# fulliu/lc

Measured on AMD Instinct MI355X. Metric: poses/sec (cov-loss fwd+bwd + weighted PnP), B=256 N=64, 1/2/4/8 MI355X, higher is better.
Workload: dtype f64; 1 GPU; configs[1]: synthetic B=256 N=64 2D-3D correspondences per GPU, HIP weighted-PnP + cov-loss; global_batch=256, n_points=64, launch=graph_region, launch_agreed_by_all_ranks=True

## Files before the change

### lc_amd/csrc/lc_common.h

```cpp
#pragma once
#include <hip/hip_runtime.h>

namespace lc {

#ifndef LC_NT_GRAD_STORES
#define LC_NT_GRAD_STORES 1
#endif
typedef float lc_v4f_t __attribute__((ext_vector_type(4)));
__device__ __forceinline__ void store_stream4(float* q, float a, float b, float c, float d) {
#if LC_NT_GRAD_STORES
    lc_v4f_t r = {a, b, c, d};
    __builtin_nontemporal_store(r, reinterpret_cast<lc_v4f_t*>(q));
#else
    *reinterpret_cast<float4*>(q) = make_float4(a, b, c, d);
#endif
}


constexpr int kWave = 64;

constexpr int kDppQuadXor1 = 0xB1;
constexpr int kDppQuadXor2 = 0x4E;
constexpr int kDppIdentity = 0xE4;
constexpr int kDppRowMirror = 0x140;
// ... 210 lines not shown
#pragma unroll
    for (int k = 0; k < K; ++k) v[k] = tot[k];
}

constexpr int kSplitMaxParts = 8;
#ifndef LC_SPLIT_WAIT_US
#define LC_SPLIT_WAIT_US 2000
#endif
constexpr unsigned long long kSplitWaitTicks = 100ull * LC_SPLIT_WAIT_US;
__device__ __forceinline__ bool split_wait_expired(int polls, unsigned long long& t0) {
    if ((polls & 15) != 15) return false;
    const unsigned long long now = __builtin_amdgcn_s_memrealtime();
    if (t0 == 0) { t0 = now; return false; }
    return now - t0 > kSplitWaitTicks;
}
constexpr int kSplitRowWords = 64;
constexpr size_t kSplitPoseBytes = 2 * kSplitMaxParts * kSplitRowWords * sizeof(unsigned long long) + 128;
constexpr int kSplitLdsDoubles = 128 + 64 + 2;
constexpr int kSplitSerialLdsDoubles = 128 + 32 * kSplitMaxParts + 32;
struct SplitSum {
    unsigned long long* exch;
    unsigned* epoch;
    int G, part;
    unsigned base;
    unsigned seq;
    bool timed_out;
};
__device__ __forceinline__ unsigned* split_tail(void* region, size_t region_bytes) {
    return reinterpret_cast<unsigned*>(static_cast<char*>(region) + region_bytes - 128);
}
__device__ __forceinline__ SplitSum split_sum_enter(void* pose_region, int G, int part) {
    unsigned* epoch = split_tail(pose_region, kSplitPoseBytes);
    return SplitSum{reinterpret_cast<unsigned long long*>(pose_region), epoch, G, part, xcd_load(epoch), 0u, false};
}
__device__ __forceinline__ void split_sum_leave(const SplitSum& sx) {
    if (sx.timed_out) xcd_store(sx.epoch + 1, 1u);
    else if (sx.part == 0 && sx.seq > 0) xcd_store(sx.epoch, sx.base + sx.seq);
}
__device__ __forceinline__ bool split_rescue_enter(void* region, size_t region_bytes, bool redo, int tid, int threads) {
    unsigned* tail = split_tail(region, region_bytes);
    const bool dirty = xcd_load(tail + 1) != 0u;
    if (!dirty && !redo) return false;
    __syncthreads();
    if (dirty) {
        unsigned long long* w = static_cast<unsigned long long*>(region);
        for (size_t i = tid; i < (region_bytes - 128) / 8; i += threads) xcd_store(w + i, 0ull);
        if (tid < 2) xcd_store(tail + tid, 0u);
    }
    if (redo && tid == 0) xcd_store(tail + 2, xcd_load(tail + 2) + 1u);
    return redo;
}

template <int K>
__device__ __forceinline__ void block_sum_split(double (&v)[K], double* lds, int tid, int& phase, SplitSum& sx) {
    static_assert(K <= 32, "one reduce-scatter of 32");
    const int lane = tid & 63, wave = tid >> 6;
    double w[32];
#pragma unroll
    for (int k = 0; k < 32; ++k) w[k] = k < K ? v[k] : 0.0;
    wave_reduce_scatter16<32>(w, lane);
    double* part = lds;
    double* tot = lds + 128 + 32 * phase;
    int* arrived_ok = reinterpret_cast<int*>(lds + 192);
    phase ^= 1;
    if (sx.timed_out) {
#pragma unroll
        for (int k = 0; k < K; ++k) v[k] = 0.0;
        return;
    }
    if ((lane & 3) == 0) *reinterpret_cast<double2*>(part + 32 * wave + scatter16_base(lane, 2)) = make_double2(w[0], w[1]);
    __syncthreads();
    if (tid < 32) {
        const unsigned long long ticket = (unsigned long long)(sx.base + sx.seq + 1u) << 32;
        unsigned long long* rows = sx.exch + (size_t)(sx.seq & 1u) * (kSplitMaxParts * kSplitRowWords) + 2 * tid;
        {
            const unsigned long long bits = __builtin_bit_cast(unsigned long long, ((part[tid] + part[32 + tid]) + part[64 + tid]) + part[96 + tid]);
            unsigned long long* mine = rows + sx.part * kSplitRowWords;
            xcd_store(mine, ticket | (bits & 0xFFFFFFFFull));
            xcd_store(mine + 1, ticket | (bits >> 32));
        }
        unsigned long long lo[kSplitMaxParts], hi[kSplitMaxParts];
        bool ok = true;
        unsigned long long t0 = 0;
        for (int polls = 0;; ++polls) {
#pragma unroll
            for (int g = 0; g < kSplitMaxParts; ++g)
                if (g < sx.G) {
                    lo[g] = xcd_load(rows + g * kSplitRowWords);
                    hi[g] = xcd_load(rows + g * kSplitRowWords + 1);
                }
            unsigned long long late = 0;
#pragma unroll
            for (int g = 0; g < kSplitMaxParts; ++g)
                if (g < sx.G) late |= ((lo[g] ^ ticket) | (hi[g] ^ ticket)) >> 32;
            if (late == 0) break;
            if (split_wait_expired(polls, t0)) { ok = false; break; }
            __builtin_amdgcn_s_sleep(1);
        }
        double s = 0.0;
#pragma unroll
        for (int g = 0; g < kSplitMaxParts; ++g)
            if (g < sx.G) s += __builtin_bit_cast(double, (hi[g] << 32) | (lo[g] & 0xFFFFFFFFull));
        tot[tid] = s;
        if (!ok) *arrived_ok = 0;
    }
    __syncthreads();
    if (!*arrived_ok) sx.timed_out = true;
#pragma unroll
    for (int k = 0; k < K; ++k) v[k] = tot[k];
    ++sx.seq;
}

template <int K>
__device__ __forceinline__ void block_sum_parts_serial(double (&v)[K], double* lds, int tid, int g, int G) {
    static_assert(K <= 32, "one reduce-scatter of 32");
    const int lane = tid & 63, wave = tid >> 6;
    double w[32];
#pragma unroll
    for (int k = 0; k < 32; ++k) w[k] = k < K ? v[k] : 0.0;
    wave_reduce_scatter16<32>(w, lane);
    double* part = lds;
    double* rows = lds + 128;
    double* tot = lds + 128 + 32 * kSplitMaxParts;
    if ((lane & 3) == 0) *reinterpret_cast<double2*>(part + 32 * wave + scatter16_base(lane, 2)) = make_double2(w[0], w[1]);
    __syncthreads();
    if (tid < 32) {
        rows[32 * g + tid] = ((part[tid] + part[32 + tid]) + part[64 + tid]) + part[96 + tid];
        if (g == G - 1) {
            double s = 0.0;
            for (int h = 0; h < G; ++h) s += rows[32 * h + tid];
            tot[tid] = s;
        }
    }
    __syncthreads();
    if (g == G - 1) {
#pragma unroll
        for (int k = 0; k < K; ++k) v[k] = tot[k];
    }
}

#ifndef LC_HORNER_ASM
#define LC_HORNER_ASM 1
#endif
__device__ __forceinline__ double horner_step(double p, double z, double c) {
#if LC_HORNER_ASM
    double r;
    asm("v_fma_f64 %0, %1, %2, %3" : "=v"(r) : "v"(p), "v"(z), "v"(c));
    return r;
#else
    return __builtin_fma(p, z, c);
#endif
}

__device__ __forceinline__ void sincos_small(double x, double& s, double& c) {
    if (!(x < 1.0e4)) {
        sincos(x, &s, &c);
        return;
    }
    const double kf = __builtin_rint(x * 0.63661977236758134308);
    const int q = (int)kf;
    double r = __builtin_fma(-kf, 1.57079632673412561417e+00, x);
    r = __builtin_fma(-kf, 6.07710050650619224932e-11, r);
    r = __builtin_fma(-kf, 2.02226624879595063154e-21, r);
    const double z = r * r;
    double ps = horner_step(1.58969099521155010221e-10, z, -2.50507602534068634195e-08);
    ps = horner_step(ps, z, 2.75573137070700676789e-06);
    ps = horner_step(ps, z, -1.98412698298579493134e-04);
    ps = horner_step(ps, z, 8.33333333332248946124e-03);
    ps = horner_step(ps, z, -1.66666666666666324348e-01);
    const double sr = __builtin_fma(ps * z, r, r);
    double pc = horner_step(-1.13596475577881948265e-11, z, 2.08757232129817482790e-09);
    pc = horner_step(pc, z, -2.75573143513906633035e-07);
    pc = horner_step(pc, z, 2.48015872894767294178e-05);
    pc = horner_step(pc, z, -1.38888888888741095749e-03);
    pc = horner_step(pc, z, 4.16666666666666019037e-02);
    const double cr = __builtin_fma(pc * z, z, __builtin_fma(-0.5, z, 1.0));
    const double ss = (q & 1) ? cr : sr, cc = (q & 1) ? sr : cr;
    s = (q & 2) ? -ss : ss;
    c = ((q + 1) & 2) ? -cc : cc;
}

__device__ __forceinline__ double atan_ratio_pos(double s, double c) {
    const bool swap = s > c;
    const double a = swap ? c : s, b = swap ? s : c;
    double t = a * fast_rcp(b);
#pragma unroll
    for (int k = 0; k < 2; ++k) {
        const double h = fast_sqrt(__builtin_fma(t, t, 1.0));
        t = t * fast_rcp(1.0 + h);
    }
    const double w = t * t;
    double p = horner_step(-1.0 / 21.0, w, 1.0 / 19.0);
    p = horner_step(p, w, -1.0 / 17.0);
    p = horner_step(p, w, 1.0 / 15.0);
    p = horner_step(p, w, -1.0 / 13.0);
    p = horner_step(p, w, 1.0 / 11.0);
    p = horner_step(p, w, -1.0 / 9.0);
    p = horner_step(p, w, 1.0 / 7.0);
    p = horner_step(p, w, -1.0 / 5.0);
    p = horner_step(p, w, 1.0 / 3.0);
    const double at = 4.0 * __builtin_fma(-(p * w), t, t);
    return swap ? 1.57079632679489661923 - at : at;
}

__device__ __forceinline__ bool uniform(bool c) { return __builtin_amdgcn_ballot_w64(c) != 0ull; }

__host__ __device__ constexpr int tri6(int i, int j) { return i * 6 - (i * (i - 1)) / 2 + (j - i); }

}
```

### lc_amd/csrc/lc_fused_kernel.h

```cpp
#pragma once
#include "lc_loss_body.h"
#include "lc_pnp_body.h"

#ifndef LC_UNIT_PRIO
#define LC_UNIT_PRIO 1
#endif

#ifndef LC_UNIT_ATTR
#define LC_UNIT_ATTR
#endif

namespace lc {
namespace {

union __attribute__((aligned(16))) FusedShared {
    loss::LossShared loss;
    double bc[pnp::kPnpLdsDoubles<1>];
};

template <int WPS>
__global__ __launch_bounds__(64, WPS) LC_UNIT_ATTR void lc_pose_unit_kernel(const LossParams lp, const PnpParams pp) {
    __shared__ FusedShared sh;
    if ((int)blockIdx.x < pp.B) {
#if LC_UNIT_PRIO
        __builtin_amdgcn_s_setprio(3);
#endif
        pnp::solve_pose<true, 1>(pp, blockIdx.x, threadIdx.x, sh.bc);
    } else {
#ifndef LC_UNIT_NOLOSS
        loss::sample<true>(lp, (int)blockIdx.x - pp.B, sh.loss);
#endif
    }
}

}

int launch_pose_unit_latency(const LossParams& lp, const PnpParams& pp, int blocks, hipStream_t stream);

}
```

### lc_amd/csrc/lc_pnp.hip

```cpp
#include "lc_pnp_kernels.h"

namespace lc {
namespace {


#ifndef LC_BIG_LOWREG
#define LC_BIG_LOWREG 0
#endif
#if LC_BIG_LOWREG
template <bool OPTS = false>
__global__ __launch_bounds__(64, 3) void lc_pnp_lm_big_kernel(const PnpParams p) {
    __shared__ __attribute__((aligned(16))) double bc[pnp::kPnpLowregLdsDoubles];
    pnp::solve_pose_lowreg<OPTS>(p, blockIdx.x, threadIdx.x, bc);
}
#endif

template <bool REG, bool OPTS = false, int PPT = 0, bool TAIL = false>
__global__ __launch_bounds__(256) void lc_pnp_lm_wide_kernel(const PnpParams p) {
    __shared__ __attribute__((aligned(16))) double bc[pnp::kPnpLdsDoubles<4>];
    pnp::solve_pose<REG, 4, false, OPTS, PPT, TAIL>(p, blockIdx.x, threadIdx.x, bc);
}

__global__ __launch_bounds__(256) void lc_pnp_lm_chain_kernel(const PnpParams a, const PnpParams b, const int second_starts_from_first) {
    __shared__ __attribute__((aligned(16))) double bc[pnp::kPnpLdsDoubles<4>];
    __shared__ float refined[8];
    pnp::solve_pose<false, 4, false, true, 4>(a, (int)(blockIdx.x % (unsigned)a.B), threadIdx.x, bc, blockIdx.x < (unsigned)a.B, refined);
    __syncthreads();
    pnp::solve_pose<false, 4, false, true, 4>(b, blockIdx.x, threadIdx.x, bc, true, nullptr, second_starts_from_first ? refined : nullptr);
}

template <bool OPTS>
__global__ __launch_bounds__(256) void lc_pnp_lm_split_kernel(const PnpParams p) {
    __shared__ __attribute__((aligned(16))) double bc[kSplitLdsDoubles];
    const int xcd = (int)(blockIdx.x % 8u), j = (int)(blockIdx.x / 8u);
    const int part = j % p.split_parts, b = (j / p.split_parts) * 8 + xcd;
    if (b >= p.B) return;
    SplitSum sx = split_sum_enter(static_cast<char*>(p.split_ws) + (size_t)b * kSplitPoseBytes, p.split_parts, part);
    if (threadIdx.x == 0) *reinterpret_cast<int*>(bc + 192) = 1;
    pnp::solve_pose<false, 4, false, OPTS, 8, true, 1>(p, b, threadIdx.x, bc, part == 0, nullptr, nullptr, &sx);
    if (threadIdx.x == 0) split_sum_leave(sx);
}

template <bool OPTS>
__global__ __launch_bounds__(256) void lc_pnp_lm_split_rescue_kernel(const PnpParams p) {
    __shared__ __attribute__((aligned(16))) double bc[kSplitSerialLdsDoubles];
    const int b = (int)blockIdx.x;
    char* region = static_cast<char*>(p.split_ws) + (size_t)b * kSplitPoseBytes;
    const bool redo = __hip_atomic_load(p.rets + b, __ATOMIC_RELAXED, __HIP_MEMORY_SCOPE_AGENT) == kPnpPartNeverArrived;
    if (!split_rescue_enter(region, kSplitPoseBytes, redo, (int)threadIdx.x, 256)) return;
    SplitSum sx{nullptr, nullptr, p.split_parts, 0, 0u, 0u, false};
    pnp::solve_pose<false, 4, false, OPTS, 0, false, 2>(p, b, threadIdx.x, bc, true, nullptr, nullptr, &sx);
}

__global__ __launch_bounds__(64, 1) void lc_pnp_lm_trace_kernel(const PnpParams p) {
    __shared__ __attribute__((aligned(16))) double bc[pnp::kPnpLdsDoubles<1>];
    pnp::solve_pose<true, 1, true>(p, blockIdx.x, threadIdx.x, bc);
}
__global__ __launch_bounds__(256) void lc_pnp_lm_wide_trace_kernel(const PnpParams p) {
    __shared__ __attribute__((aligned(16))) double bc[pnp::kPnpLdsDoubles<4>];
    pnp::solve_pose<false, 4, true>(p, blockIdx.x, threadIdx.x, bc);
}

}

int launch_pnp_lm_trace(const PnpParams& p, hipStream_t stream) {
    if (p.B <= 0) return 0;
    if (p.Nmax <= 64) hipLaunchKernelGGL(lc_pnp_lm_trace_kernel, dim3(p.B), dim3(64), 0, stream, p);
    else hipLaunchKernelGGL(lc_pnp_lm_wide_trace_kernel, dim3(p.B), dim3(256), 0, stream, p);
    return hipGetLastError() == hipSuccess ? 0 : 2;
}

int launch_pnp_lm_chain(const PnpParams& a, const PnpParams& b, hipStream_t stream) {
    const auto wide4 = [](const PnpParams& p) { return p.Nmax > 256 && p.Nmax <= 1024; };
    const float* b_start = b.start ? b.start : b.states;
    const bool rows_match = b_start != a.states || b.pose_mod == a.B || (b.pose_mod == 0 && b.B == a.B);
    const bool first_is_safe = a.start != nullptr || b.B == a.B;
    if (a.B > 0 && b.B > 0 && a.Nmax <= 64 && b.Nmax <= 64 && b.B <= kLatencyGridMax && b.B % a.B == 0 && rows_match && first_is_safe)
        return launch_pnp_lm_chain_latency(a, b, b_start == a.states ? 1 : 0, stream);
    if (a.B > 0 && b.B > 0 && wide4(a) && wide4(b) && b.B % a.B == 0 && rows_match && first_is_safe) {
        hipLaunchKernelGGL(lc_pnp_lm_chain_kernel, dim3(b.B), dim3(256), 0, stream, a, b, b_start == a.states ? 1 : 0);
        return hipGetLastError() == hipSuccess ? 0 : 2;
    }
    if (int rc = launch_pnp_lm(a, stream)) return rc;
    return launch_pnp_lm(b, stream);
}

int device_compute_units() {
    static int cached[64] = {};
    int dev = 0, n = 0;
    if (hipGetDevice(&dev) != hipSuccess) return 0;
    if (dev >= 0 && dev < 64 && cached[dev]) return cached[dev];
    if (hipDeviceGetAttribute(&n, hipDeviceAttributeMultiprocessorCount, dev) != hipSuccess) return 0;
    if (dev >= 0 && dev < 64) cached[dev] = n;
    return n;
}
int split_parts_for(int units) {
    const int cus = device_compute_units();
    for (int parts = 8; parts >= 2; parts >>= 1)
        if ((long long)units * parts <= cus) return parts;
    return 1;
}

int pnp_split_parts(int B, int Nmax) {
    if (Nmax <= kSplitMinPoints || B <= 0) return 1;
    return split_parts_for((B + 7) / 8 * 8);
}
size_t pnp_split_workspace_bytes(int B, int Nmax) { return pnp_split_parts(B, Nmax) > 1 ? (size_t)B * kSplitPoseBytes : 0; }

int launch_pnp_lm(const PnpParams& p, hipStream_t stream) {
    if (p.B <= 0) return 0;
    if (p.split_ws && p.split_parts > 1) {
        const dim3 grid((unsigned)((p.B + 7) / 8 * 8 * p.split_parts));
        if (p.options || p.weight_mask || p.pose_mod > 0) {
            hipLaunchKernelGGL(lc_pnp_lm_split_kernel<true>, grid, dim3(256), 0, stream, p);
            hipLaunchKernelGGL(lc_pnp_lm_split_rescue_kernel<true>, dim3((unsigned)p.B), dim3(256), 0, stream, p);
        } else {
            hipLaunchKernelGGL(lc_pnp_lm_split_kernel<false>, grid, dim3(256), 0, stream, p);
            hipLaunchKernelGGL(lc_pnp_lm_split_rescue_kernel<false>, dim3((unsigned)p.B), dim3(256), 0, stream, p);
        }
        return hipGetLastError() == hipSuccess ? 0 : 2;
    }
    const bool big = p.B > kLatencyGridMax;
    if (p.options || p.weight_mask || p.pose_mod > 0) {
        if (p.Nmax <= 64) {
#if LC_BIG_LOWREG
            if (big) hipLaunchKernelGGL(lc_pnp_lm_big_kernel<true>, dim3(p.B), dim3(64), 0, stream, p);
#else
            if (big) hipLaunchKernelGGL((lc_pnp_lm_kernel<true, LC_BIG_WPS, true>), dim3(p.B), dim3(64), 0, stream, p);
#endif
            else return launch_pnp_lm_latency(p, stream);
        } else if (p.Nmax <= 256) {
            hipLaunchKernelGGL((lc_pnp_lm_wide_kernel<true, true>), dim3(p.B), dim3(256), 0, stream, p);
        } else if (p.Nmax <= 1024) {
            hipLaunchKernelGGL((lc_pnp_lm_wide_kernel<false, true, 4>), dim3(p.B), dim3(256), 0, stream, p);
        } else if (p.Nmax <= 2048) {
            hipLaunchKernelGGL((lc_pnp_lm_wide_kernel<false, true, 8>), dim3(p.B), dim3(256), 0, stream, p);
        } else {
            hipLaunchKernelGGL((lc_pnp_lm_wide_kernel<false, true, 16, true>), dim3(p.B), dim3(256), 0, stream, p);
        }
        return hipGetLastError() == hipSuccess ? 0 : 2;
    }
    if (p.Nmax <= 64) {
#if LC_BIG_LOWREG
        if (big) hipLaunchKernelGGL(lc_pnp_lm_big_kernel<false>, dim3(p.B), dim3(64), 0, stream, p);
#else
        if (big) hipLaunchKernelGGL((lc_pnp_lm_kernel<true, LC_BIG_WPS>), dim3(p.B), dim3(64), 0, stream, p);
#endif
        else return launch_pnp_lm_latency(p, stream);
    } else if (p.Nmax <= 256) {
        hipLaunchKernelGGL(lc_pnp_lm_wide_kernel<true>, dim3(p.B), dim3(256), 0, stream, p);
    } else if (p.Nmax <= 1024) {
        hipLaunchKernelGGL((lc_pnp_lm_wide_kernel<false, false, 4>), dim3(p.B), dim3(256), 0, stream, p);
    } else if (p.Nmax <= 2048) {
        hipLaunchKernelGGL((lc_pnp_lm_wide_kernel<false, false, 8>), dim3(p.B), dim3(256), 0, stream, p);
    } else {
        hipLaunchKernelGGL((lc_pnp_lm_wide_kernel<false, false, 16, true>), dim3(p.B), dim3(256), 0, stream, p);
    }
    return hipGetLastError() == hipSuccess ? 0 : 2;
}

}
```

### lc_amd/csrc/lc_pnp_body.h

```cpp
#pragma once
#include <cfloat>

#include "lc_common.h"
#include "lc_kernels.h"

#ifdef LC_STAMPS
#define LC_PSTAMP_DECL unsigned long long pst_[8] = {0, 0, 0, 0, 0, 0, 0, 0}, pt0_ = 0, pt1_ = 0
#define LC_PSTAMP_BEGIN()                                                                 \
    do {                                                                                  \
        __builtin_amdgcn_sched_barrier(0);                                                \
        asm volatile("s_memtime %0\n\ts_waitcnt lgkmcnt(0)" : "=s"(pt0_)::"memory");      \
        __builtin_amdgcn_sched_barrier(0);                                                \
    } while (0)
#define LC_PSTAMP(i)                                                                      \
    do {                                                                                  \
        __builtin_amdgcn_sched_barrier(0);                                                \
        asm volatile("s_memtime %0\n\ts_waitcnt lgkmcnt(0)" : "=s"(pt1_)::"memory");      \
        __builtin_amdgcn_sched_barrier(0);                                                \
        pst_[i] += pt1_ - pt0_;                                                           \
        pt0_ = pt1_;                                                                      \
    } while (0)
#else
#define LC_PSTAMP_DECL
#define LC_PSTAMP_BEGIN() do {} while (0)
#define LC_PSTAMP(i) do {} while (0)
#endif

#ifndef LC_WIDE_REG_SUM_REGS
#define LC_WIDE_REG_SUM_REGS 1
#endif
#ifndef LC_PNP_STREAM_SUM
#define LC_PNP_STREAM_SUM 1
#endif

namespace lc {
namespace pnp {

template <int NW>
constexpr int kPnpLdsDoubles = sum_bcast_lds_doubles<NW>(28);

struct Point {
    double X[3];
    double u, v;
    double a, b, c;
};

struct Rot {
    double R[9];
    double Jr[9];
};

__device__ __forceinline__ void make_rot(const double aa[3], Rot& o) {
    const double x = aa[0], y = aa[1], z = aa[2];
    const double th2 = x * x + y * y + z * z;
    const bool small = !(th2 > DBL_EPSILON);
    double th, ith;
    fast_sqrt_rsqrt(th2, th, ith);
    double s, c;
    sincos_small(th, s, c);
    const double ith2 = ith * ith;
    const double A = small ? 1.0 : s * ith;
    const double B = small ? 0.0 : (1.0 - c) * ith2;
    const double C = small ? 0.0 : (th - s) * ith2 * ith;
    const double cd = small ? 1.0 : c;
    o.R[0] = cd + B * x * x;    o.R[1] = B * x * y - A * z; o.R[2] = B * x * z + A * y;
    o.R[3] = B * x * y + A * z; o.R[4] = cd + B * y * y;    o.R[5] = B * y * z - A * x;
    o.R[6] = B * x * z - A * y; o.R[7] = B * y * z + A * x; o.R[8] = cd + B * z * z;
    const double d = 1.0 - C * th2;
    o.Jr[0] = d + C * x * x;     o.Jr[1] = C * x * y + B * z; o.Jr[2] = C * x * z - B * y;
    o.Jr[3] = C * x * y - B * z; o.Jr[4] = d + C * y * y;     o.Jr[5] = C * y * z + B * x;
    o.Jr[6] = C * x * z + B * y; o.Jr[7] = C * y * z - B * x; o.Jr[8] = d + C * z * z;
}

template <bool FIRST, bool STREAM = false, int NW = 1>
__device__ __forceinline__ void accumulate_point(const Point& pt, const Rot& rt, const double t[3], const double k[6],
                                                 const double (&sc)[6], double (&acc)[28], double* lds = nullptr, int pos = 0) {
    double rx[3], q[3];
#pragma unroll
    for (int d = 0; d < 3; ++d) {
        rx[d] = rt.R[3 * d] * pt.X[0] + rt.R[3 * d + 1] * pt.X[1] + rt.R[3 * d + 2] * pt.X[2];
        q[d] = rx[d] + t[d];
    }
    const double iz = fast_rcp(q[2]);
    const double up = (q[0] * k[0] + q[1] * k[1]) * iz, vp = (q[0] * k[3] + q[1] * k[4]) * iz;
    const double du = up - pt.u, dv = vp - pt.v;
    const double r[2] = {du * pt.a + dv * pt.b, dv * pt.c};
    const double dup[3] = {k[0] * iz, k[1] * iz, -up * iz};
    const double dvp[3] = {k[3] * iz, k[4] * iz, -vp * iz};
    double J[2][6];
#pragma unroll
    for (int m = 0; m < 3; ++m) {
        J[0][3 + m] = pt.a * dup[m] + pt.b * dvp[m];
        J[1][3 + m] = pt.c * dvp[m];
    }
#pragma unroll
    for (int rr = 0; rr < 2; ++rr) {
        double cr[3];
        cr[0] = rx[1] * J[rr][5] - rx[2] * J[rr][4];
        cr[1] = rx[2] * J[rr][3] - rx[0] * J[rr][5];
        cr[2] = rx[0] * J[rr][4] - rx[1] * J[rr][3];
#pragma unroll
        for (int m = 0; m < 3; ++m) J[rr][m] = (rt.Jr[3 * m] * cr[0] + rt.Jr[3 * m + 1] * cr[1] + rt.Jr[3 * m + 2] * cr[2]) * sc[m];
#pragma unroll
        for (int m = 0; m < 3; ++m) J[rr][3 + m] *= sc[3 + m];
    }
#pragma unroll
    for (int i = 0; i < 6; ++i) {
#pragma unroll
        for (int j = i; j < 6; ++j) {
            const double v = __builtin_fma(J[0][i], J[0][j], J[1][i] * J[1][j]);
            if constexpr (STREAM) block_sum_put<NW>(lds, pos, tri6(i, j), v);
            else acc[tri6(i, j)] = FIRST ? v : acc[tri6(i, j)] + v;
        }
        const double gi = __builtin_fma(J[0][i], r[0], J[1][i] * r[1]);
        if constexpr (STREAM) block_sum_put<NW>(lds, pos, 21 + i, gi);
        else acc[21 + i] = FIRST ? gi : acc[21 + i] + gi;
    }
    const double ss = __builtin_fma(r[0], r[0], r[1] * r[1]);
    if constexpr (STREAM) block_sum_put<NW>(lds, pos, 27, ss);
    else acc[27] = FIRST ? ss : acc[27] + ss;
}

__device__ __forceinline__ bool ldlt_solve6(const double (&A)[21], const double (&dg)[6], const double (&rhs)[6], double (&y)[6]) {
    double L[6][6], Ld[6][6], id[6];
    bool ok = true;
#pragma unroll
    for (int j = 0; j < 6; ++j) {
        double dj = A[tri6(j, j)] + dg[j];
#pragma unroll
        for (int k = 0; k < j; ++k) dj -= L[j][k] * Ld[j][k];
        ok = ok && (dj > 0) && (dj < DBL_MAX);
        id[j] = fast_rcp(dj);
#pragma unroll
        for (int i = j + 1; i < 6; ++i) {
            double v = A[tri6(j, i)];
#pragma unroll
            for (int k = 0; k < j; ++k) v -= L[i][k] * Ld[j][k];
            Ld[i][j] = v;
            L[i][j] = v * id[j];
        }
    }
    double z[6];
#pragma unroll
    for (int i = 0; i < 6; ++i) {
        double v = rhs[i];
#pragma unroll
        for (int k = 0; k < i; ++k) v -= L[i][k] * z[k];
        z[i] = v;
    }
#pragma unroll
    for (int i = 5; i >= 0; --i) {
        double v = z[i] * id[i];
#pragma unroll
        for (int k = i + 1; k < 6; ++k) v -= L[k][i] * y[k];
        y[i] = v;
    }
    return ok;
}

struct RawPoint {
    float X[3];
    float2 u;
    float a, b, c;
};
__device__ __forceinline__ float nan_to_num(float f) { return f != f ? 0.f : fminf(fmaxf(f, -FLT_MAX), FLT_MAX); }

template <bool OPTS = false>
__device__ __forceinline__ RawPoint load_raw_point(const PnpParams& p, size_t base, int n) {
    RawPoint o;
    const float* X = p.pts3d + (base + n) * 3;
    o.u = *reinterpret_cast<const float2*>(p.pts2d + (base + n) * 2);
    o.X[0] = X[0]; o.X[1] = X[1]; o.X[2] = X[2];
    if (OPTS && p.weight_mask) {
        const float m = p.weight_mask[base + n] ? 1.f : 0.f;
        o.a = m; o.b = 0.f; o.c = m;
    } else if (p.sqrtL) {
        const float4 L = *reinterpret_cast<const float4*>(p.sqrtL + (base + n) * 4);
        o.a = L.x; o.b = L.z; o.c = L.w;
    } else {
        const float2 L = *reinterpret_cast<const float2*>(p.sqrt_diag + (base + n) * 2);
        o.a = L.x; o.b = 0.f; o.c = L.y;
    }
    if constexpr (OPTS) {
        if (p.options & kPnpWeightsAreStd) { o.a = 1.f / (o.a * o.a); o.c = 1.f / (o.c * o.c); }
        if (p.options & kPnpNanToNum) {
            o.u.x = nan_to_num(o.u.x); o.u.y = nan_to_num(o.u.y);
            o.X[0] = nan_to_num(o.X[0]); o.X[1] = nan_to_num(o.X[1]); o.X[2] = nan_to_num(o.X[2]);
            o.a = nan_to_num(o.a); o.b = nan_to_num(o.b); o.c = nan_to_num(o.c);
        }
        if (p.options & kPnpWeightsAreIcov) { o.a = sqrtf(o.a); o.c = sqrtf(o.c); }
    }
    return o;
}
__device__ __forceinline__ Point to_point(const RawPoint& r, const double cam[6]) {
    Point o;
    o.X[0] = r.X[0]; o.X[1] = r.X[1]; o.X[2] = r.X[2];
    o.u = (double)r.u.x - cam[2];
    o.v = (double)r.u.y - cam[5];
    o.a = r.a; o.b = r.b; o.c = r.c;
    return o;
}
template <bool OPTS = false>
__device__ __forceinline__ Point load_point(const PnpParams& p, size_t base, int n, const double cam[6]) {
    return to_point(load_raw_point<OPTS>(p, base, n), cam);
}

__device__ __forceinline__ double max_abs6(const double (&v)[6]) {
    double m = 0;
#pragma unroll
    for (int j = 0; j < 6; ++j) m = fmax(m, fabs(v[j]));
    return m;
}
__device__ __forceinline__ double norm6(const double (&v)[6]) {
    double m = 0;
#pragma unroll
    for (int j = 0; j < 6; ++j) m += v[j] * v[j];
    return fast_sqrt(m);
}

template <bool REG, int NW = 1, bool TRACE = false, bool OPTS = false, int PPT = 0, bool TAIL = false, int SPLIT = 0>
__device__ __forceinline__ void solve_pose(const PnpParams& p, int b, int lane, double* bc, bool store = true, float* handoff = nullptr,
                                           const float* start_override = nullptr, [[maybe_unused]] SplitSum* sx = nullptr) {
    constexpr int kThreads = kWave * NW;
    static_assert(SPLIT != 1 || (NW == 4 && !REG && PPT > 0 && !TRACE), "the split form is the four-wave cached-prefix solve");
    static_assert(SPLIT != 2 || (NW == 4 && !REG && PPT == 0 && !TRACE), "the rescue form walks memory, part by part");
    const int slot = SPLIT == 1 ? lane + kThreads * sx->part : lane;
    const int stride = SPLIT == 1 ? kThreads * sx->G : kThreads;
#ifdef LC_TRACE_CLOCK
    const unsigned long long t_start_ = __builtin_amdgcn_s_memtime();
#endif
    LC_PSTAMP_DECL;
    LC_PSTAMP_BEGIN();
    const int n = p.counts ? p.counts[b] : p.Nmax;
    const int bk = (OPTS && p.pose_mod > 0) ? b % p.pose_mod : b;
    const float* st_in = start_override ? start_override : (p.start ? p.start + 7 * (size_t)bk : p.states + 7 * (size_t)b);
    const bool filter = OPTS && (p.options & kPnpNanToNum);
    auto fin = [&](float f) { return filter ? nan_to_num(f) : f; };
    if (n < 3) {
        if (lane == 0 && store) {
            p.rets[b] = 1;
            p.result_tr[b] = 1.f;
            if (p.iters) p.iters[b] = 0;
        }
        if (lane < 7) {
            const float v = fin(st_in[lane]);
            if (store && (p.start || start_override || filter)) p.states[7 * (size_t)b + lane] = v;
            if (handoff) handoff[lane] = v;
        }
        return;
    }
    const size_t base = (size_t)b * p.Nmax;
    const bool active = lane < n;
    RawPoint raw;
    if constexpr (REG) raw = load_raw_point<OPTS>(p, base, active ? lane : 0);
    [[maybe_unused]] RawPoint rawc[PPT > 0 ? PPT : 1];
    if constexpr (!REG && PPT > 0) {
#pragma unroll
        for (int k = 0; k < PPT; ++k)
            if (slot + k * stride < n) rawc[k] = load_raw_point<OPTS>(p, base, slot + k * stride);
    }
    double cam[6];
    {
        const float* Kp = p.K + 9 * (size_t)bk;
#pragma unroll
        for (int i = 0; i < 6; ++i) cam[i] = fin(Kp[i]);
    }
    double x[6];
    {
        float stf[7];
#pragma unroll
        for (int i = 0; i < 7; ++i) stf[i] = st_in[i];
        asm volatile("" : "+v"(stf[0]), "+v"(stf[1]), "+v"(stf[2]), "+v"(stf[3]), "+v"(stf[4]), "+v"(stf[5]), "+v"(stf[6]));
        const double q0 = fin(stf[0]), q1 = fin(stf[1]), q2 = fin(stf[2]), q3 = fin(stf[3]);
        const double s2 = q1 * q1 + q2 * q2 + q3 * q3;
        double kk = 2.0;
        if (s2 > 0.0) {
            const double s = fast_sqrt(s2);
            const double half = atan_ratio_pos(s, fabs(q0));
            const double two_theta = 2.0 * ((q0 < 0.0) ? -half : half);
            kk = two_theta / s;
        }
        x[0] = q1 * kk; x[1] = q2 * kk; x[2] = q3 * kk;
        x[3] = fin(stf[4]); x[4] = fin(stf[5]); x[5] = fin(stf[6]);
    }
    LC_PSTAMP(0);
    Point rp;
    if constexpr (REG) {
        rp = to_point(raw, cam);
        if (!active) { rp.a = 0.0; rp.b = 0.0; rp.c = 0.0; }
    }

    [[maybe_unused]] int sum_phase = 0;
    auto evaluate = [&](const double (&xe)[6], const double (&sc)[6], double (&H)[21], double (&g)[6], double& cost) -> bool {
        LC_PSTAMP(1);
        Rot rt;
        make_rot(xe, rt);
        LC_PSTAMP(2);
        const double t[3] = {xe[3], xe[4], xe[5]};
        double acc[28];
        if constexpr (REG && LC_PNP_STREAM_SUM && !(NW == 4 && LC_WIDE_REG_SUM_REGS)) {
            const int pos = block_sum_open<NW>(lane);
            accumulate_point<true, true, NW>(rp, rt, t, cam, sc, acc, bc, pos);
            LC_PSTAMP(3);
            block_sum_close<28, NW>(acc, bc, lane);
        } else if constexpr (REG) {
            accumulate_point<true>(rp, rt, t, cam, sc, acc);
            LC_PSTAMP(3);
            if constexpr (NW == 4 && LC_WIDE_SUM_REGS) block_sum_waves4<28>(acc, bc, lane, sum_phase);
            else block_sum_bcast_lds<28, NW>(acc, bc, lane);
        } else {
#pragma unroll
            for (int i = 0; i < 28; ++i) acc[i] = 0;
            if constexpr (PPT > 0) {
#pragma unroll
                for (int k = 0; k < PPT; ++k)
                    if (slot + k * stride < n) accumulate_point<false>(to_point(rawc[k], cam), rt, t, cam, sc, acc);
                if constexpr (TAIL)
                    for (int i = slot + PPT * stride; i < n; i += stride) accumulate_point<false>(load_point<OPTS>(p, base, i, cam), rt, t, cam, sc, acc);
            } else if constexpr (SPLIT == 2) {
                for (int g = 0; g < sx->G; ++g) {
                    if (g > 0) {
#pragma unroll
                        for (int i = 0; i < 28; ++i) acc[i] = 0;
                    }
                    for (int i = lane + kThreads * g; i < n; i += kThreads * sx->G) accumulate_point<false>(load_point<OPTS>(p, base, i, cam), rt, t, cam, sc, acc);
                    block_sum_parts_serial<28>(acc, bc, lane, g, sx->G);
                }
            } else {
                for (int i = lane; i < n; i += kThreads) accumulate_point<false>(load_point<OPTS>(p, base, i, cam), rt, t, cam, sc, acc);
            }
            LC_PSTAMP(3);
            if constexpr (SPLIT == 2) {}
            else if constexpr (SPLIT == 1) block_sum_split<28>(acc, bc, lane, sum_phase, *sx);
            else if constexpr (NW == 4 && LC_WIDE_SUM_REGS) block_sum_waves4<28>(acc, bc, lane, sum_phase);
            else block_sum_bcast_lds<28, NW>(acc, bc, lane);
        }
        LC_PSTAMP(4);
#pragma unroll
        for (int i = 0; i < 21; ++i) H[i] = acc[i];
#pragma unroll
        for (int i = 0; i < 6; ++i) g[i] = acc[21 + i];
        const double ss = acc[27];
        cost = 0.5 * ss;
        double chk = ss;
#pragma unroll
        for (int i = 0; i < 6; ++i) chk += H[tri6(i, i)];
        LC_PSTAMP(5);
        if constexpr (SPLIT == 1) {
            if (sx->timed_out) return false;
        }
        return chk <= DBL_MAX;
    };

    const double ftol = p.ftol, ptol = 1e-8, gtol = 1e-10;
    double H[21], g[6], cost;
    double scale[6], iscale[6];
    bool failed;
    {
        const double one[6] = {1, 1, 1, 1, 1, 1};
        failed = !evaluate(x, one, H, g, cost);
#pragma unroll
        for (int j = 0; j < 6; ++j) {
            iscale[j] = 1.0 + fast_sqrt(H[tri6(j, j)]);
            scale[j] = fast_rcp(iscale[j]);
        }
#pragma unroll
        for (int i = 0; i < 6; ++i) {
#pragma unroll
            for (int j = i; j < 6; ++j) H[tri6(i, j)] *= scale[i] * scale[j];
            g[i] *= scale[i];
        }
    }
    auto grad_max = [&](const double (&gs)[6]) {
        double m = 0;
#pragma unroll
        for (int j = 0; j < 6; ++j) m = fmax(m, fabs(gs[j]) * iscale[j]);
        return m;
    };
    double gmax = grad_max(g);
    auto sqnorm6 = [](const double (&v)[6]) {
        double m = 0;
#pragma unroll
        for (int j = 0; j < 6; ++j) m += v[j] * v[j];
        return m;
    };
    double xn2 = sqnorm6(x);
    double radius = 1e4, dfac = 2.0;
    int iter = 0, n_invalid = 0;
    bool converged = false;
    auto trace = [&](int kind, double cost_x, double cost_cand, double mcc, double rho, double step_norm) {
        if constexpr (TRACE) {
            if (lane == 0 && p.trace && iter <= p.trace_rows) {
                double* row = p.trace + ((size_t)b * p.trace_rows + (iter - 1)) * 8;
                row[0] = kind; row[1] = cost_x; row[2] = cost_cand; row[3] = mcc; row[4] = rho; row[5] = step_norm;
                row[6] = radius; row[7] = gmax;
#ifdef LC_TRACE_CLOCK
                row[7] = (double)(__builtin_amdgcn_s_memtime() - t_start_);
#endif
            }
        }
    };

    while (uniform(!failed && !converged)) {
        if (iter >= p.max_iter) break;
        if (uniform(gmax <= gtol || radius <= 1e-32)) { converged = true; break; }
        ++iter;
        double dg[6], y[6];
        const double inv_radius = fast_rcp(radius);
#pragma unroll
        for (int i = 0; i < 6; ++i) dg[i] = fmin(fmax(H[tri6(i, i)], 1e-6), 1e32) * inv_radius;
        LC_PSTAMP(1);
        bool step_ok = ldlt_solve6(H, dg, g, y);
        LC_PSTAMP(6);
        double mcc = 0;
#pragma unroll
        for (int i = 0; i < 6; ++i) mcc += y[i] * (g[i] + dg[i] * y[i]);
        mcc *= 0.5;
        step_ok = step_ok && (mcc > 0.0) && (mcc <= DBL_MAX);
        if (uniform(!step_ok)) {
            if (++n_invalid >= 5) { failed = true; trace(0, cost, 0.0, mcc, 0.0, 0.0); break; }
            radius /= dfac; dfac *= 2.0;
            trace(0, cost, 0.0, mcc, 0.0, 0.0);
            continue;
        }
        n_invalid = 0;
        double xc[6], delta[6];
#pragma unroll
        for (int j = 0; j < 6; ++j) { delta[j] = -y[j] * scale[j]; xc[j] = x[j] + delta[j]; }
        const double sn2 = sqnorm6(delta);
        const bool ptol_in_reach = TRACE || uniform(!(sn2 > 2.0 * ptol * ptol * (xn2 + ptol * ptol)));
        double step_norm = 0.0;
        bool ptol_hit = false;
        if (ptol_in_reach) {
            step_norm = fast_sqrt(sn2);
            ptol_hit = uniform(step_norm <= ptol * (fast_sqrt(xn2) + ptol));
        }
        double cost_c;
        const bool cand_ok = evaluate(xc, scale, H, g, cost_c);
        if constexpr (SPLIT == 1) {
            if (sx->timed_out) { failed = true; break; }
        }
        if (!cand_ok) cost_c = DBL_MAX;
        if (ptol_hit) {
            converged = true; trace(3, cost, cost_c, mcc, 0.0, step_norm); break;
        }
        const double cost_change = cost - cost_c;
        if (uniform(fabs(cost_change) <= ftol * cost)) {
            converged = true; trace(4, cost, cost_c, mcc, cost_change * fast_rcp(mcc), step_norm); break;
        }
        const double rel = cost_change * fast_rcp(mcc);
        if (uniform(rel > 1e-3)) {
#pragma unroll
            for (int j = 0; j < 6; ++j) x[j] = xc[j];
            const double cost_prev = cost;
            cost = cost_c;
            xn2 = sqnorm6(x);
            gmax = grad_max(g);
            const double tq = 2.0 * rel - 1.0;
            radius = fmin(1e16, radius * fast_rcp(fmax(1.0 / 3.0, 1.0 - tq * tq * tq)));
            dfac = 2.0;
            trace(1, cost_prev, cost_c, mcc, rel, step_norm);
        } else {
            radius /= dfac; dfac *= 2.0;
            trace(2, cost, cost_c, mcc, rel, step_norm);
            double cost_again;
            if (!evaluate(x, scale, H, g, cost_again)) { failed = true; break; }
        }
    }
    LC_PSTAMP(1);
#ifdef LC_STAMPS
    if (lane == 0 && p.iters) {
        unsigned long long* o = reinterpret_cast<unsigned long long*>(p.iters) + 8 * (size_t)b;
        for (int i = 0; i < 6; ++i) o[i] = pst_[i];
        o[6] = iter;
        o[7] = pst_[6];
    }
#endif
    const bool invalid = failed || !converged;
    if (invalid && lane < 7) {
        const float v = fin(st_in[lane]);
        if (store && (p.start || start_override || filter)) p.states[7 * (size_t)b + lane] = v;
        if (handoff) handoff[lane] = v;
    }
    if (lane == 0) {
        if (store) {
            p.rets[b] = invalid ? 1 : 0;
            if constexpr (SPLIT == 1) {
                if (sx->timed_out) p.rets[b] = kPnpPartNeverArrived;
            }
            p.result_tr[b] = (float)radius;
#ifndef LC_STAMPS
            if (p.iters) p.iters[b] = iter;
#endif
        }
        if (!invalid) {
            float stq[7];
            float* st = stq;
            const double t2 = x[0] * x[0] + x[1] * x[1] + x[2] * x[2];
            double q0 = 1.0, kk = 0.5;
            if (t2 > 0.0) {
                const double th = fast_sqrt(t2), h = 0.5 * th;
                double sh, ch;
                sincos_small(h, sh, ch);
                q0 = ch;
                kk = sh / th;
            }
            st[0] = (float)q0; st[1] = (float)(x[0] * kk); st[2] = (float)(x[1] * kk); st[3] = (float)(x[2] * kk);
            st[4] = (float)x[3]; st[5] = (float)x[4]; st[6] = (float)x[5];
#pragma unroll
            for (int k = 0; k < 7; ++k) {
                if (store) p.states[7 * (size_t)b + k] = stq[k];
                if (handoff) handoff[k] = stq[k];
            }
        }
    }
}


constexpr int kPnpLowregLdsDoubles = kPnpLdsDoubles<1> + 30;

__device__ __forceinline__ bool ldlt_solve6_lds(const double* A, const double* g, double inv_radius, double (&y)[6], double& mcc) {
    double L[6][6], Ld[6][6], id[6];
    bool ok = true;
    auto dgv = [&](int i) { return fmin(fmax(A[tri6(i, i)], 1e-6), 1e32) * inv_radius; };
#pragma unroll
    for (int j = 0; j < 6; ++j) {
        double dj = A[tri6(j, j)] + dgv(j);
#pragma unroll
        for (int k = 0; k < j; ++k) dj -= L[j][k] * Ld[j][k];
        ok = ok && (dj > 0) && (dj < DBL_MAX);
        id[j] = fast_rcp(dj);
#pragma unroll
        for (int i = j + 1; i < 6; ++i) {
            double v = A[tri6(j, i)];
#pragma unroll
            for (int k = 0; k < j; ++k) v -= L[i][k] * Ld[j][k];
            Ld[i][j] = v;
            L[i][j] = v * id[j];
        }
    }
    double z[6];
#pragma unroll
    for (int i = 0; i < 6; ++i) {
        double v = g[i];
#pragma unroll
        for (int k = 0; k < i; ++k) v -= L[i][k] * z[k];
        z[i] = v;
    }
#pragma unroll
    for (int i = 5; i >= 0; --i) {
        double v = z[i] * id[i];
#pragma unroll
        for (int k = i + 1; k < 6; ++k) v -= L[k][i] * y[k];
        y[i] = v;
    }
// ... 216 lines not shown
```

### lc_amd/csrc/lc_pnp_kernels.h

```cpp
#pragma once
#include "lc_pnp_body.h"

namespace lc {
namespace {

template <bool REG, int WPS, bool OPTS = false>
__global__ __launch_bounds__(64, WPS) void lc_pnp_lm_kernel(const PnpParams p) {
    __shared__ __attribute__((aligned(16))) double bc[pnp::kPnpLdsDoubles<1>];
    pnp::solve_pose<REG, 1, false, OPTS>(p, blockIdx.x, threadIdx.x, bc);
}

}

int launch_pnp_lm_latency(const PnpParams& p, hipStream_t stream);
int launch_pnp_lm_chain_latency(const PnpParams& a, const PnpParams& b, int second_starts_from_first, hipStream_t stream);

}
```

### lc_amd/csrc/lc_pnp_latency.hip

```cpp
#include "lc_pnp_kernels.h"

namespace lc {

namespace {
__global__ __launch_bounds__(64, 1) void lc_pnp_lm_chain_small_kernel(const PnpParams a, const PnpParams b, const int second_starts_from_first) {
    __shared__ __attribute__((aligned(16))) double bc[pnp::kPnpLdsDoubles<1>];
    __shared__ float refined[8];
    pnp::solve_pose<true, 1, false, true>(a, (int)(blockIdx.x % (unsigned)a.B), threadIdx.x, bc, blockIdx.x < (unsigned)a.B, refined);
    __syncthreads();
    pnp::solve_pose<true, 1, false, true>(b, blockIdx.x, threadIdx.x, bc, true, nullptr, second_starts_from_first ? refined : nullptr);
}
}

int launch_pnp_lm_chain_latency(const PnpParams& a, const PnpParams& b, int second_starts_from_first, hipStream_t stream) {
    hipLaunchKernelGGL(lc_pnp_lm_chain_small_kernel, dim3(b.B), dim3(64), 0, stream, a, b, second_starts_from_first);
    return hipGetLastError() == hipSuccess ? 0 : 2;
}

int launch_pnp_lm_latency(const PnpParams& p, hipStream_t stream) {
    if (p.options || p.weight_mask || p.pose_mod > 0) hipLaunchKernelGGL((lc_pnp_lm_kernel<true, 1, true>), dim3(p.B), dim3(64), 0, stream, p);
    else hipLaunchKernelGGL((lc_pnp_lm_kernel<true, 1>), dim3(p.B), dim3(64), 0, stream, p);
    return hipGetLastError() == hipSuccess ? 0 : 2;
}

}
```

Baseline: 19.79 million poses/s.

## Add flat single-region LM loop and branch-free sincos for one-wave PnP solve

Adds a FLAT variant of the one-wave register PnP Levenberg-Marquardt loop. It evaluates the candidate and computes the next-step quantities (gradient max, radius, norms) speculatively before any uniform branch, and puts all the rare exits (invalid step, rejection, convergence) behind one combined uniform check. The aim is to cut the divergent control flow and serial dependency chain in each iteration. It also adds sincos_small_flat, which always runs the reduced polynomial and calls a noinline cold libm sincos only when some lane has a large argument. In exchange, the fast path does extra work speculatively, and the rejection and restart logic is duplicated in a way that must stay consistent with the original loop.

```diff
diff --git a/lc_amd/csrc/lc_common.h b/lc_amd/csrc/lc_common.h
--- a/lc_amd/csrc/lc_common.h
+++ b/lc_amd/csrc/lc_common.h
@@ -386,11 +386,28 @@
 #endif
 }
 
+__device__ __forceinline__ void sincos_reduced(double x, double& s, double& c);
 __device__ __forceinline__ void sincos_small(double x, double& s, double& c) {
     if (!(x < 1.0e4)) {
         sincos(x, &s, &c);
         return;
     }
+    sincos_reduced(x, s, c);
+}
+__device__ __attribute__((noinline, cold)) double2 sincos_libm_cold(double x) {
+    double s, c;
+    sincos(x, &s, &c);
+    return make_double2(s, c);
+}
+__device__ __forceinline__ void sincos_small_flat(double x, double& s, double& c) {
+    sincos_reduced(x, s, c);
+    if (__builtin_expect(__builtin_amdgcn_ballot_w64(!(x < 1.0e4)) != 0ull, 0)) {
+        const double2 sc = sincos_libm_cold(x);
+        s = sc.x;
+        c = sc.y;
+    }
+}
+__device__ __forceinline__ void sincos_reduced(double x, double& s, double& c) {
     const double kf = __builtin_rint(x * 0.63661977236758134308);
     const int q = (int)kf;
     double r = __builtin_fma(-kf, 1.57079632673412561417e+00, x);
diff --git a/lc_amd/csrc/lc_fused_kernel.h b/lc_amd/csrc/lc_fused_kernel.h
--- a/lc_amd/csrc/lc_fused_kernel.h
+++ b/lc_amd/csrc/lc_fused_kernel.h
@@ -25,7 +25,7 @@
 #if LC_UNIT_PRIO
         __builtin_amdgcn_s_setprio(3);
 #endif
-        pnp::solve_pose<true, 1>(pp, blockIdx.x, threadIdx.x, sh.bc);
+        pnp::solve_pose<true, 1, false, false, 0, false, 0, WPS == 1>(pp, blockIdx.x, threadIdx.x, sh.bc);
     } else {
 #ifndef LC_UNIT_NOLOSS
         loss::sample<true>(lp, (int)blockIdx.x - pp.B, sh.loss);
diff --git a/lc_amd/csrc/lc_pnp.hip b/lc_amd/csrc/lc_pnp.hip
--- a/lc_amd/csrc/lc_pnp.hip
+++ b/lc_amd/csrc/lc_pnp.hip
@@ -54,7 +54,7 @@
 
 __global__ __launch_bounds__(64, 1) void lc_pnp_lm_trace_kernel(const PnpParams p) {
     __shared__ __attribute__((aligned(16))) double bc[pnp::kPnpLdsDoubles<1>];
-    pnp::solve_pose<true, 1, true>(p, blockIdx.x, threadIdx.x, bc);
+    pnp::solve_pose<true, 1, true, false, 0, false, 0, true>(p, blockIdx.x, threadIdx.x, bc);
 }
 __global__ __launch_bounds__(256) void lc_pnp_lm_wide_trace_kernel(const PnpParams p) {
     __shared__ __attribute__((aligned(16))) double bc[pnp::kPnpLdsDoubles<4>];
diff --git a/lc_amd/csrc/lc_pnp_body.h b/lc_amd/csrc/lc_pnp_body.h
--- a/lc_amd/csrc/lc_pnp_body.h
+++ b/lc_amd/csrc/lc_pnp_body.h
@@ -50,6 +50,7 @@
     double Jr[9];
 };
 
+template <bool FLAT = false>
 __device__ __forceinline__ void make_rot(const double aa[3], Rot& o) {
     const double x = aa[0], y = aa[1], z = aa[2];
     const double th2 = x * x + y * y + z * z;
@@ -57,7 +58,8 @@
     double th, ith;
     fast_sqrt_rsqrt(th2, th, ith);
     double s, c;
-    sincos_small(th, s, c);
+    if constexpr (FLAT) sincos_small_flat(th, s, c);
+    else sincos_small(th, s, c);
     const double ith2 = ith * ith;
     const double A = small ? 1.0 : s * ith;
     const double B = small ? 0.0 : (1.0 - c) * ith2;
@@ -218,12 +220,13 @@
     return fast_sqrt(m);
 }
 
-template <bool REG, int NW = 1, bool TRACE = false, bool OPTS = false, int PPT = 0, bool TAIL = false, int SPLIT = 0>
+template <bool REG, int NW = 1, bool TRACE = false, bool OPTS = false, int PPT = 0, bool TAIL = false, int SPLIT = 0, bool FLAT = false>
 __device__ __forceinline__ void solve_pose(const PnpParams& p, int b, int lane, double* bc, bool store = true, float* handoff = nullptr,
                                            const float* start_override = nullptr, [[maybe_unused]] SplitSum* sx = nullptr) {
     constexpr int kThreads = kWave * NW;
     static_assert(SPLIT != 1 || (NW == 4 && !REG && PPT > 0 && !TRACE), "the split form is the four-wave cached-prefix solve");
     static_assert(SPLIT != 2 || (NW == 4 && !REG && PPT == 0 && !TRACE), "the rescue form walks memory, part by part");
+    static_assert(!FLAT || (REG && NW == 1 && SPLIT == 0), "the one-region loop is the one-wave register solve's");
     const int slot = SPLIT == 1 ? lane + kThreads * sx->part : lane;
     const int stride = SPLIT == 1 ? kThreads * sx->G : kThreads;
 #ifdef LC_TRACE_CLOCK
@@ -294,7 +297,7 @@
     auto evaluate = [&](const double (&xe)[6], const double (&sc)[6], double (&H)[21], double (&g)[6], double& cost) -> bool {
         LC_PSTAMP(1);
         Rot rt;
-        make_rot(xe, rt);
+        make_rot<FLAT>(xe, rt);
         LC_PSTAMP(2);
         const double t[3] = {xe[3], xe[4], xe[5]};
         double acc[28];
@@ -364,13 +367,16 @@
             iscale[j] = 1.0 + fast_sqrt(H[tri6(j, j)]);
             scale[j] = fast_rcp(iscale[j]);
         }
+    }
+    auto jacobi_scale = [&]() {
 #pragma unroll
         for (int i = 0; i < 6; ++i) {
 #pragma unroll
             for (int j = i; j < 6; ++j) H[tri6(i, j)] *= scale[i] * scale[j];
             g[i] *= scale[i];
         }
-    }
+    };
+    jacobi_scale();
     auto grad_max = [&](const double (&gs)[6]) {
         double m = 0;
 #pragma unroll
@@ -401,6 +407,107 @@
         }
     };
 
+    if constexpr (FLAT) {
+        auto head_stops = [&]() -> bool {
+            if (iter >= p.max_iter) return true;
+            if (uniform(gmax <= gtol || radius <= 1e-32)) { converged = true; return true; }
+            return false;
+        };
+        bool from_start = true;
+        if (uniform(!failed) && !head_stops()) for (;;) {
+            ++iter;
+            double dg[6], y[6];
+            const double inv_radius = fast_rcp(radius);
+#pragma unroll
+            for (int i = 0; i < 6; ++i) dg[i] = fmin(fmax(H[tri6(i, i)], 1e-6), 1e32) * inv_radius;
+            LC_PSTAMP(1);
+            bool step_ok = ldlt_solve6(H, dg, g, y);
+            LC_PSTAMP(6);
+            double mcc = 0;
+#pragma unroll
+            for (int i = 0; i < 6; ++i) mcc += y[i] * (g[i] + dg[i] * y[i]);
+            mcc *= 0.5;
+            step_ok = step_ok && (mcc > 0.0) && (mcc <= DBL_MAX);
+            double xc[6], delta[6];
+#pragma unroll
+            for (int j = 0; j < 6; ++j) { delta[j] = -y[j] * scale[j]; xc[j] = x[j] + delta[j]; }
+            const double sn2 = sqnorm6(delta);
+            const bool ptol_in_reach = !(sn2 > 2.0 * ptol * ptol * (xn2 + ptol * ptol));
+            [[maybe_unused]] double step_norm = 0.0;
+            bool ptol_flag = ptol_in_reach;
+            if constexpr (TRACE) {
+                step_norm = fast_sqrt(sn2);
+                ptol_flag = step_norm <= ptol * (fast_sqrt(xn2) + ptol);
+            }
+            double cost_c;
+            const bool cand_ok = evaluate(xc, scale, H, g, cost_c);
+            if (!cand_ok) cost_c = DBL_MAX;
+            const double cost_change = cost - cost_c;
+            const bool ftol_hit = fabs(cost_change) <= ftol * cost;
+            const double rel = cost_change * fast_rcp(mcc);
+            const bool accept = rel > 1e-3;
+            const double xn2_n = sqnorm6(xc);
+            const double gmax_n = grad_max(g);
+            const double tq = 2.0 * rel - 1.0;
+            const double radius_n = fmin(1e16, radius * fast_rcp(fmax(1.0 / 3.0, 1.0 - tq * tq * tq)));
+            const bool stops_n = (gmax_n <= gtol) | (radius_n <= 1e-32);
+            bool more = true;
+            if (uniform(!step_ok | ptol_flag | ftol_hit | !accept | stops_n) | (iter >= p.max_iter)) {
+                const bool invalid_step = uniform(!step_ok);
+                bool rejected = false;
+                if (invalid_step) {
+                    if (++n_invalid >= 5) { failed = true; trace(0, cost, 0.0, mcc, 0.0, 0.0); break; }
+                    radius /= dfac; dfac *= 2.0;
+                    trace(0, cost, 0.0, mcc, 0.0, 0.0);
+                } else {
+                    n_invalid = 0;
+                    bool ptol_hit = false;
+                    if constexpr (TRACE) ptol_hit = uniform(ptol_flag);
+                    else if (uniform(ptol_in_reach)) ptol_hit = uniform(fast_sqrt(sn2) <= ptol * (fast_sqrt(xn2) + ptol));
+                    if (ptol_hit) {
+                        converged = true; trace(3, cost, cost_c, mcc, 0.0, step_norm); break;
+                    }
+                    if (uniform(ftol_hit)) {
+                        converged = true; trace(4, cost, cost_c, mcc, rel, step_norm); break;
+                    }
+                    rejected = !uniform(accept);
+                    if (rejected) {
+                        radius /= dfac; dfac *= 2.0;
+                        trace(2, cost, cost_c, mcc, rel, step_norm);
+                    } else {
+                        more = !(uniform(stops_n) | (iter >= p.max_iter));
+                        if (!more && iter < p.max_iter) converged = true;
+                    }
+                }
+                if (invalid_step || rejected) {
+                    const bool unit = invalid_step && from_start;
+                    double sc[6], cost_again;
+#pragma unroll
+                    for (int j = 0; j < 6; ++j) sc[j] = unit ? 1.0 : scale[j];
+                    const bool ok = evaluate(x, sc, H, g, cost_again);
+                    if (unit) jacobi_scale();
+                    if (rejected) {
+                        if (!ok) { failed = true; break; }
+                        from_start = false;
+                    }
+                    if (head_stops()) break;
+                    continue;
+                }
+            }
+            n_invalid = 0;
+#pragma unroll
+            for (int j = 0; j < 6; ++j) x[j] = xc[j];
+            const double cost_prev = cost;
+            cost = cost_c;
+            xn2 = xn2_n;
+            gmax = gmax_n;
+            radius = radius_n;
+            dfac = 2.0;
+            from_start = false;
+            trace(1, cost_prev, cost_c, mcc, rel, step_norm);
+            if (!more) break;
+        }
+    } else
     while (uniform(!failed && !converged)) {
         if (iter >= p.max_iter) break;
         if (uniform(gmax <= gtol || radius <= 1e-32)) { converged = true; break; }
diff --git a/lc_amd/csrc/lc_pnp_kernels.h b/lc_amd/csrc/lc_pnp_kernels.h
--- a/lc_amd/csrc/lc_pnp_kernels.h
+++ b/lc_amd/csrc/lc_pnp_kernels.h
@@ -7,7 +7,7 @@
 template <bool REG, int WPS, bool OPTS = false>
 __global__ __launch_bounds__(64, WPS) void lc_pnp_lm_kernel(const PnpParams p) {
     __shared__ __attribute__((aligned(16))) double bc[pnp::kPnpLdsDoubles<1>];
-    pnp::solve_pose<REG, 1, false, OPTS>(p, blockIdx.x, threadIdx.x, bc);
+    pnp::solve_pose<REG, 1, false, OPTS, 0, false, 0, REG && WPS == 1>(p, blockIdx.x, threadIdx.x, bc);
 }
 
 }
diff --git a/lc_amd/csrc/lc_pnp_latency.hip b/lc_amd/csrc/lc_pnp_latency.hip
--- a/lc_amd/csrc/lc_pnp_latency.hip
+++ b/lc_amd/csrc/lc_pnp_latency.hip
@@ -6,9 +6,9 @@
 __global__ __launch_bounds__(64, 1) void lc_pnp_lm_chain_small_kernel(const PnpParams a, const PnpParams b, const int second_starts_from_first) {
     __shared__ __attribute__((aligned(16))) double bc[pnp::kPnpLdsDoubles<1>];
     __shared__ float refined[8];
-    pnp::solve_pose<true, 1, false, true>(a, (int)(blockIdx.x % (unsigned)a.B), threadIdx.x, bc, blockIdx.x < (unsigned)a.B, refined);
+    pnp::solve_pose<true, 1, false, true, 0, false, 0, true>(a, (int)(blockIdx.x % (unsigned)a.B), threadIdx.x, bc, blockIdx.x < (unsigned)a.B, refined);
     __syncthreads();
-    pnp::solve_pose<true, 1, false, true>(b, blockIdx.x, threadIdx.x, bc, true, nullptr, second_starts_from_first ? refined : nullptr);
+    pnp::solve_pose<true, 1, false, true, 0, false, 0, true>(b, blockIdx.x, threadIdx.x, bc, true, nullptr, second_starts_from_first ? refined : nullptr);
 }
 }
 
```

Result: slower. 19.41 million poses/s (-1.9%).
